# CHONSPQX/modulated-deform-conv

Hardware: AMD Instinct MI355X
Metric: fwd+bwd GSamples/s, MDCN2d 3x3 C=256 56x56 B=32; %HBM roofline (higher is better)
Workload: dtype f32; 1 GPU; ModulatedDeformConv2d 3x3, C_in=C_out=256, 56x56, deformable_group=1, fp32, B=32 per GPU, forward+backward (BASELINE.json configs[1]); global_batch=32, parallelism=dp1 batch-sharded

## Files before the change

modulated_deform_conv_amd/csrc/mfma_bwd_data.hip:

```cpp
#include "mfma_kernels.hpp"
#include "mfma_tile.hpp"
#include <algorithm>
#include <map>
#include <mutex>
#include <stdio.h>
#include <stdlib.h>

namespace mdconv {

namespace {

int grid_for(int64_t total) {
  int64_t b = (total + 255) / 256;
  return (int)(b > 8192 ? 8192 : (b < 1 ? 1 : b));
}

__device__ __forceinline__ void pack_wq_items(const Geom &g, int ochunks, int cblks, const float *__restrict__ w,
                                              float *__restrict__ wq, int64_t first, int64_t step) {
  const int64_t total = (int64_t)g.K * ochunks * cblks * 2 * 64;
  for (int64_t i = first; i < total; i += step) {
    int64_t r = i;
    const int lane = (int)(r & 63); r >>= 6;
    const int q = (int)(r & 1); r >>= 1;
    const int cblk = (int)(r % cblks); r /= cblks;
// ... 957 lines not shown
        }
      }
    }
    if (step > 0) {
      float *tp = tile + (r * 4) * (QT + 1) + (a - q0);
      tp[0] = cur.x; tp[QT + 1] = cur.y; tp[2 * (QT + 1)] = cur.z; tp[3 * (QT + 1)] = cur.w;
    }
    cur = nxt;
    nxt = make_float4(0.f, 0.f, 0.f, 0.f);
  }
  __syncthreads();
  for (int x = threadIdx.x; x < CW * (QT / 8); x += 256) {
    const int c = x / (QT / 8), qs8 = (x % (QT / 8)) * 8;
    float *dst = grad_input + ((int64_t)b * g.C + c) * g.S_i + q0 + qs8;
    const float *src = tile + c * (QT + 1) + qs8;
#pragma unroll
    for (int k = 0; k < 8; ++k)
      if (q0 + qs8 + k < g.S_i) dst[k] = g.acc_data ? dst[k] + src[k] : src[k];
  }
}

}

int pack_wq_f32(const Geom &g, const BwdDims &bd, const float *weight, float *wq, hipStream_t stream) {
  const int64_t total = (int64_t)g.K * bd.ochunks * bd.cblks_q * 2 * 64;
  hipLaunchKernelGGL(pack_wq_kernel, dim3(grid_for(total)), dim3(256), 0, stream, g, bd.ochunks,
                     bd.cblks_q, weight, wq);
  return check_launch("pack_wq");
}

int bwd_prep_f32(const Geom &g, const BwdDims &bd, const float *weight, float *wq, int *cnt, const float *x,
                 float *xt, hipStream_t stream) {
  const int64_t pack_total = (int64_t)g.K * bd.ochunks * bd.cblks_q * 2 * 64;
  const int64_t cnt_n = (int64_t)g.B * g.DG * bd.S_e;
  int nb_pack = grid_for(pack_total), nb_zero = grid_for(cnt_n);
  if (nb_pack > 512) nb_pack = 512;
  if (nb_zero > 256) nb_zero = 256;
  const int qtiles = (g.S_i + 31) / 32, ctiles = g.C / 32;
  const int64_t nb_t = xt ? (int64_t)qtiles * ctiles * g.B : 0;
  if (nb_t + nb_pack + nb_zero > 0x7fffffff) {
    int rc = pack_wq_f32(g, bd, weight, wq, stream);
    if (!rc) rc = csr_zero_f32(g, bd, cnt, stream);
    if (!rc && xt) rc = nchw_to_nhwc_f32(g, x, xt, stream);
    return rc;
  }
  hipLaunchKernelGGL(bwd_prep_kernel, dim3((unsigned)(nb_pack + nb_zero + nb_t)), dim3(256), 0, stream, g, bd.ochunks,
                     bd.cblks_q, weight, wq, cnt, cnt_n, x, xt, nb_pack, nb_zero, qtiles, ctiles);
  return check_launch("bwd_prep");
}

int num_cus() {
  static int n = 0;
  if (n == 0) {
    int dev = 0, v = 0;
    if (hipGetDevice(&dev) == hipSuccess &&
        hipDeviceGetAttribute(&v, hipDeviceAttributeMultiprocessorCount, dev) == hipSuccess && v > 0)
      n = v;
    else
      n = 256;
  }
  return n;
}

size_t bwd_data_lds_bytes(const Geom &g, const BwdDims &bd) {
  const int bnp = 32 * (4 / bd.waves_c);
  const int passes = bd.cblks_q / (2 * bd.waves_c);
  const size_t red = (size_t)bd.red_floats;
// ... 48 lines not shown
                       dim3(256), lds, stream,                                                  \
                       g, bd, (const float *)t.input, (const float *)t.grad_output, wq,         \
                       (const float *)t.offset, (const float *)t.mask, gcol,                    \
                       (float *)t.grad_offset, (float *)t.grad_mask, ga, bias_part, cnt, table, xt,        \
                       ntiles, n_full, n_tail, tpw);                                            \
  } while (0)
                                                \
#define LAUNCH_BD(ND, MOD, WC, QPQ)                                                             \
  do {                                                                                          \
    if (xt != nullptr && bd.cl_drain) LAUNCH_BD_(ND, MOD, WC, QPQ, true);                       \
    else LAUNCH_BD_(ND, MOD, WC, QPQ, false);                                                   \
  } while (0)
#define LAUNCH_BD2(ND, MOD)                                                                     \
  do {                                                                                          \
    const int nbatch = ND == 2 ? 4 : 8, nquads = bd.ochunks / 4;                                \
                   \
    const int qpq = (ND == 2 && g.G == 1 && nquads % nbatch == 0 && nquads / nbatch <= 2) ? nquads / nbatch : 0; \
    if (bd.waves_c == 4) {                                                                      \
      if (ND == 2 && qpq == 1) LAUNCH_BD(ND, MOD, 4, (ND == 2 ? 1 : 0));                        \
      else if (ND == 2 && qpq == 2) LAUNCH_BD(ND, MOD, 4, (ND == 2 ? 2 : 0));                   \
      else LAUNCH_BD(ND, MOD, 4, 0);                                                            \
    } else if (bd.waves_c == 2) LAUNCH_BD(ND, MOD, 2, 0);                                       \
    else LAUNCH_BD(ND, MOD, 1, 0);                                                              \
  } while (0)
  if (g.nd == 2) { if (g.modulated) LAUNCH_BD2(2, true); else LAUNCH_BD2(2, false); }
  else { if (g.modulated) LAUNCH_BD2(3, true); else LAUNCH_BD2(3, false); }
#undef LAUNCH_BD2
#undef LAUNCH_BD
#undef LAUNCH_BD_
  return check_launch("mfma_bwd_data");
}

int csr_zero_f32(const Geom &g, const BwdDims &bd, int *cnt, hipStream_t stream) {
  const int64_t cnt_n = (int64_t)g.B * g.DG * bd.S_e;
  hipLaunchKernelGGL(zero_int_kernel, dim3(grid_for(cnt_n)), dim3(256), 0, stream, cnt, cnt_n);
  return check_launch("zero_cnt");
}

int csr_build_f32(const Geom &g, const BwdDims &bd, const Tensors &t, int *cnt, int *rowptr,
                  void *entries, hipStream_t stream) {
  const int64_t samples = (int64_t)g.B * g.DG * g.K * g.S_o;
  int rc;
  hipLaunchKernelGGL(csr_scan_kernel, dim3((bd.S_e + kScanChunk - 1) / kScanChunk, g.B * g.DG), dim3(256), 0,
                     stream, bd.S_e, cnt, rowptr);
  if ((rc = check_launch("csr_scan"))) return rc;
  if (bd.sample_keyed) return csr_fill3d_f32(g, bd, t, cnt, rowptr, entries, stream);
#define LAUNCH_CSR(ND, MOD)                                                                     \
  hipLaunchKernelGGL((csr_fill_kernel<ND, MOD>), dim3(grid_for(samples)), dim3(256), 0, stream,  \
                     g, (const float *)t.offset, (const float *)t.mask, cnt, rowptr,            \
                     (int4 *)entries)
  if (g.modulated) LAUNCH_CSR(2, true); else LAUNCH_CSR(2, false);
#undef LAUNCH_CSR
  return check_launch("csr_fill");
}

int col2im_f32(const Geom &g, const BwdDims &bd, const Tensors &t, const float *gcol,
               const int *rowptr, const void *entries, float *sums, hipStream_t stream) {
  if (bd.sample_keyed) return col2im3d_f32(g, bd, t, gcol, rowptr, entries, sums, stream);
  const int qtiles = (g.S_i + 31) / 32;
  const dim3 grid(g.B * qtiles, 1);
#define LAUNCH_GG(ND, LPD)                                                                      \
  hipLaunchKernelGGL((col2im_gather_grouped_kernel<ND, LPD>), grid, dim3(256), 0, stream, g,    \
                     gcol, rowptr, (const int4 *)entries, (float *)t.grad_input)
#define LAUNCH_NARROW(ND, LPD)                                                                  \
  do {                                                                                          \
    const int qt = 4 * (64 / LPD) * kRun;                                                       \
    hipLaunchKernelGGL((col2im_gather_narrow_kernel<ND, LPD>), dim3(g.B * ((g.S_i + qt - 1) / qt)), \
// ... 22 lines not shown
```

modulated_deform_conv_amd/csrc/mfma_bwd_weight.hip:

```cpp
#include "mfma_kernels.hpp"
#include "mfma_tile.hpp"

namespace mdconv {

namespace {


template <int ND, bool PADN, int WR, int WC, int MB>
__global__ __launch_bounds__(256) void mfma_bwd_weight_kernel(Geom g, BwdDims bd,
                                                              const float *__restrict__ input,
                                                              const float *__restrict__ ga,
                                                              const int *__restrict__ table,
                                                              float *__restrict__ part) {
  static_assert(WR * WC == 4, "four waves");
  constexpr int NC = 1 << ND, NP = NC / 2;
  constexpr int BK = kBK;
  constexpr int RM = WR * MB * 32, CN = WC * 32;
  constexpr int CT = CN / 16;
  constexpr int kPitch = CN + 1;
  __shared__ __attribute__((aligned(16))) float Bs[2 * BK * kPitch];

  int id = blockIdx.x;
  const int cblk = id % bd.cblks; id /= bd.cblks;
  const int tap = id % g.K;
  const int mtile = id / g.K;
  const int split = blockIdx.y;
  const int c0 = cblk * CN;
  const int dg = min(c0, g.C - 1) / g.Cdg;

  const int tid = threadIdx.x, lane = tid & 63, kh = lane >> 5;
  const int wave = __builtin_amdgcn_readfirstlane(tid >> 6);
  const int wr = wave / WC, wcn = wave % WC;
  const int kk = tid & 15, sub = tid >> 4;

// ... 200 lines not shown
  float s = 0.f;
#pragma unroll
  for (int k = 0; k < kBiasSlices; ++k) s += stage[(size_t)k * g.O + o];
  grad_bias[o] = g.acc_w ? grad_bias[o] + s : s;
}

int grid_for(int64_t total) {
  int64_t b = (total + 255) / 256;
  return (int)(b > 8192 ? 8192 : (b < 1 ? 1 : b));
}

}

int mfma_bwd_weight_occupancy(int nd, bool padn, int wtile) {
  static int cache[2][2][2] = {};
  int &slot = cache[nd == 3][padn][wtile == 1];
  if (slot) return slot;
  int n = 0;
#define OCC_BW(ND, PADN, WR, WC, MB)                                                                           \
  (void)hipOccupancyMaxActiveBlocksPerMultiprocessor(                                                          \
      &n, reinterpret_cast<const void *>(&mfma_bwd_weight_kernel<ND, PADN, WR, WC, MB>), 256, 0)
#define OCC_BW2(ND, PADN) OCC_BW(ND, PADN, 4, 1, 2)
  if (nd == 2) { if (padn) OCC_BW2(2, true); else OCC_BW2(2, false); }
  else { if (padn) OCC_BW2(3, true); else OCC_BW2(3, false); }
#undef OCC_BW2
#undef OCC_BW
  (void)hipGetLastError();
  if (n <= 0) n = 4;
  slot = n;
  return n;
}

int mfma_bwd_weight_f32(const Geom &g, const BwdDims &bd, const Tensors &t, const float *ga,
                        const int *table, float *part, const float *bias_part, const float *xt,
                        hipStream_t stream) {
  const dim3 grid(bd.mtiles * g.K * bd.cblks, bd.splits);
  const bool padn = bd.Np != g.N;
  profile_mark(2, true, stream, bd.cl ? "mfma_bwd_weight_cl_kernel" : "mfma_bwd_weight_kernel");
  if (bd.cl) {
    const int rcl = mfma_bwd_weight_cl_launch(g, bd, xt, ga, table, part, stream);
    if (rcl) return rcl;
  } else {
#define LAUNCH_BW(ND, PADN, WR, WC, MB)                                                         \
  hipLaunchKernelGGL((mfma_bwd_weight_kernel<ND, PADN, WR, WC, MB>), grid, dim3(256), 0, stream, \
                     g, bd, (const float *)t.input, ga, table, part)
#define LAUNCH_BW2(ND, PADN) LAUNCH_BW(ND, PADN, 4, 1, 2)
  if (g.nd == 2) { if (padn) LAUNCH_BW2(2, true); else LAUNCH_BW2(2, false); }
  else { if (padn) LAUNCH_BW2(3, true); else LAUNCH_BW2(3, false); }
#undef LAUNCH_BW2
#undef LAUNCH_BW
  }
  profile_mark(2, false, stream);
  int rc = check_launch("mfma_bwd_weight");
  if (rc) return rc;
  hipLaunchKernelGGL(reduce_weight_kernel, dim3(grid_for((int64_t)g.K * g.O * g.Cg)), dim3(256), 0,
                     stream, g, bd, part, (float *)t.grad_weight);
  return check_launch("reduce_weight");
}

size_t grad_bias_stage_bytes(const Geom &g) { return (size_t)kBiasSlices * g.O * sizeof(float); }

int grad_bias_f32(const Geom &g, const BwdDims &bd, const float *bias_part, float *stage, float *grad_bias,
                  hipStream_t stream) {
  if (!g.with_bias) return MDCONV_OK;
  hipLaunchKernelGGL(grad_bias_stage1_kernel, dim3((g.O + 63) / 64, kBiasSlices), dim3(256), 0, stream, g,
                     bd.bias_tiles, bias_part, stage);
  int rc = check_launch("grad_bias_stage1");
  if (rc) return rc;
  hipLaunchKernelGGL(grad_bias_final_kernel, dim3((g.O + 255) / 256), dim3(256), 0, stream, g, stage, grad_bias);
  return check_launch("grad_bias_final");
}

}
```

modulated_deform_conv_amd/csrc/mfma_bwd_weight_cl.hip:

```cpp
#include "mfma_kernels.hpp"
#include "mfma_tile.hpp"

#include <stdlib.h>

namespace mdconv {

namespace {


template <int ND, bool PADN, int WR, int WC, int MB, int NBW>
__global__ __launch_bounds__(256, 1) void mfma_bwd_weight_cl_kernel(Geom g, BwdDims bd,
                                                                 const float *__restrict__ xt,
                                                                 const float *__restrict__ ga,
                                                                 const int *__restrict__ table,
                                                                 float *__restrict__ part) {
  static_assert(WR * WC == 4 && WC * NBW * 32 == 64, "four waves, 64 input channels");
  constexpr int NC = 1 << ND;
  constexpr int BK = kBK;
  constexpr int RM = WR * MB * 32, CN = WC * NBW * 32;
  constexpr int NH = CN / 64;
  constexpr int kPitch = CN + 1;
  __shared__ __attribute__((aligned(16))) float Bs[2 * BK * kPitch];

  const int per_split = gridDim.x;
  const int unit = xcd_remap(blockIdx.x + per_split * blockIdx.y, per_split * gridDim.y);
  const int split = unit / per_split;
  int id = unit - split * per_split;
  const int cblk = id % bd.cblks; id /= bd.cblks;
  const int tap = id % g.K;
  const int mtile = id / g.K;
  const int c0 = cblk * CN;

  const int tid = threadIdx.x, lane = tid & 63, kh = lane >> 5;
  const int wave = __builtin_amdgcn_readfirstlane(tid >> 6);
  const int wr = wave / WC, wcn = wave % WC;
  const int cq = tid & 15, kk = tid >> 4;

  const int pairs_total = bd.Np / 32;
  const int p_begin = split * bd.pairs_per_split;
  const int p_end = min(p_begin + bd.pairs_per_split, pairs_total);
  const int t_begin = 2 * p_begin, t_end = 2 * p_end;

  const rsrc_t r_xt = make_rsrc(xt, (size_t)g.B * g.S_i * g.C * sizeof(float));
  const int slab_bytes = bd.mblks * 2 * 64 * 16;
  const rsrc_t r_ga = make_rsrc(ga, (size_t)(bd.Np / 16) * slab_bytes);
  const int entry_bytes = 2 * NC * 4;
  const int dg = c0 / g.Cdg;
  const rsrc_t r_tab = make_rsrc(table + (size_t)(dg * g.K + tap) * bd.Np * (2 * NC),
                                 (size_t)bd.Np * entry_bytes);
  const int wo = mtile * RM + wr * MB * 32;
  const int a_voff = ((wo / 32) * 2 * 64 + lane) * 16;
  bool m_active = wo < g.O;
  if (g.G > 1) {
    const int cw = c0 + wcn * NBW * 32;
    const int o_lo = (min(cw, g.C - 1) / g.Cg) * g.Og;
    const int o_hi = (min(cw + NBW * 32 - 1, g.C - 1) / g.Cg + 1) * g.Og;
    m_active = m_active && wo < o_hi && wo + MB * 32 > o_lo;
  }
  const int t_voff = kk * entry_bytes;
  const int c_voff = (min(c0, g.C - CN) + cq * 4) * 4;
// ... 72 lines not shown
    load_tab(tabA, t_begin);
    load_tab(tabB, t_begin + 1);
    load_a(ra0, t_begin);
    gather(tabA);
    for (int t = t_begin; t < t_end; t += 2) {
      commit(tabA, t, Bs);
      __syncthreads();
      load_a(ra1, t + 1);
      gather(tabB);
      load_tab(tabA, min(t + 2, t_last));
      __builtin_amdgcn_sched_barrier(0);
      mma(ra0, Bs);
      commit(tabB, t + 1, Bs + BK * kPitch);
      __syncthreads();
      load_a(ra0, min(t + 2, t_last));
      gather(tabA);
      load_tab(tabB, min(t + 3, t_last));
      __builtin_amdgcn_sched_barrier(0);
      mma(ra1, Bs + BK * kPitch);
    }
  }

#pragma unroll
  for (int n = 0; n < NBW; ++n) {
    float *dst = part + ((size_t)(split * g.K + tap) * bd.OgpB) * bd.Cp + c0 + (wcn * NBW + n) * 32 + (lane & 31);
#pragma unroll
    for (int mb = 0; mb < MB; ++mb)
#pragma unroll
      for (int r = 0; r < 16; ++r) {
        const int o = wo + mb * 32 + (r & 3) + 8 * (r >> 2) + 4 * kh;
        dst[(size_t)o * bd.Cp] = acc[mb][n][r];
      }
  }
}


template <int ND, bool PADN, int MB>
__global__ __launch_bounds__(256) void mfma_bwd_weight_cl64_kernel(Geom g, BwdDims bd,
                                                                   const float *__restrict__ xt,
                                                                   const float *__restrict__ ga,
                                                                   const int *__restrict__ table,
                                                                   float *__restrict__ part) {
  constexpr int NC = 1 << ND;
  constexpr int SW = 2 * NC;
  constexpr int SP = 64;
  constexpr int kPitch = 65;
  constexpr int RM = 2 * MB * 32;
  constexpr int TPT = (SP * SW + 1023) / 1024;
  static_assert(TPT == 1, "one table piece per thread");
  __shared__ __attribute__((aligned(16))) float Bs[2 * SP * kPitch];
  __shared__ __attribute__((aligned(16))) int Ts[2 * SP * SW];

  const int per_split = gridDim.x;
  const int unit = xcd_remap(blockIdx.x + per_split * blockIdx.y, per_split * gridDim.y);
  const int split = unit / per_split;
  int id = unit - split * per_split;
  const int cblk = id % bd.cblks; id /= bd.cblks;
  const int tap = id % g.K;
  const int mtile = id / g.K;
  const int c0 = cblk * 64;

  const int tid = threadIdx.x, lane = tid & 63, kh = lane >> 5;
  const int wave = __builtin_amdgcn_readfirstlane(tid >> 6);
  const int wr = wave >> 1, wcn = wave & 1;
  const int cq = tid & 15, pg = tid >> 4;

// ... 150 lines not shown
#define MDCONV_CL_INSTANCE(ND, PADN, CALL)                                                                     \
  do {                                                                                                          \
    if (wtile == 1) { CALL##64(ND, PADN, 1); }                                                                  \
    else if (wtile == 2) { CALL##64(ND, PADN, 2); }                                                             \
    else { CALL(ND, PADN, 4, 1, 2, 2); }                                                                        \
  } while (0)
#define MDCONV_CL_DISPATCH(CALL)                                                                               \
  do {                                                                                                          \
    if (nd == 2) { if (padn) MDCONV_CL_INSTANCE(2, true, CALL); else MDCONV_CL_INSTANCE(2, false, CALL); }      \
    else { if (padn) MDCONV_CL_INSTANCE(3, true, CALL); else MDCONV_CL_INSTANCE(3, false, CALL); }              \
  } while (0)

int mfma_bwd_weight_cl_occupancy(int nd, bool padn, int wtile) {
  static int cache[2][2][4] = {};
  int &slot = cache[nd == 3][padn][wtile < 0 || wtile > 3 ? 3 : wtile];
  if (slot) return slot;
  int n = 0;
#define OCC_CL(ND, PADN, WR, WC, MB, NBW)                                                                      \
  (void)hipOccupancyMaxActiveBlocksPerMultiprocessor(                                                          \
      &n, reinterpret_cast<const void *>(&mfma_bwd_weight_cl_kernel<ND, PADN, WR, WC, MB, NBW>), 256, 0)
#define OCC_CL64(ND, PADN, MB)                                                                                 \
  (void)hipOccupancyMaxActiveBlocksPerMultiprocessor(                                                          \
      &n, reinterpret_cast<const void *>(&mfma_bwd_weight_cl64_kernel<ND, PADN, MB>), 256, 0)
  MDCONV_CL_DISPATCH(OCC_CL);
#undef OCC_CL64
#undef OCC_CL
  (void)hipGetLastError();
  if (n <= 0) n = 3;
  slot = n;
  return n;
}

int mfma_bwd_weight_cl_launch(const Geom &g, const BwdDims &bd, const float *xt, const float *ga,
                              const int *table, float *part, hipStream_t stream) {
  const dim3 grid(bd.mtiles * g.K * bd.cblks, bd.splits);
  const bool padn = bd.Np != g.N;
  const int nd = g.nd, wtile = bd.wtile;
#define LAUNCH_CL(ND, PADN, WR, WC, MB, NBW)                                                                   \
  hipLaunchKernelGGL((mfma_bwd_weight_cl_kernel<ND, PADN, WR, WC, MB, NBW>), grid, dim3(256), 0,               \
                     stream, g, bd, xt, ga, table, part)
#define LAUNCH_CL64(ND, PADN, MB)                                                                              \
  hipLaunchKernelGGL((mfma_bwd_weight_cl64_kernel<ND, PADN, MB>), grid, dim3(256), 0, stream, g, bd, xt, ga,   \
                     table, part)
  MDCONV_CL_DISPATCH(LAUNCH_CL);
#undef LAUNCH_CL64
#undef LAUNCH_CL
  return check_launch("mfma_bwd_weight_cl");
}

#undef MDCONV_CL_DISPATCH
#undef MDCONV_CL_INSTANCE

}
```

modulated_deform_conv_amd/csrc/mfma_kernels.hip:

```cpp
#include "mfma_kernels.hpp"
#include "mfma_tile.hpp"

#include <stdio.h>
#include <stdlib.h>
#include <string.h>

#include <atomic>
#include <mutex>
#include <vector>

namespace mdconv {

namespace {

std::atomic<bool> g_prof_on{false};
std::mutex g_prof_mu;
struct ProfPair { hipEvent_t a, b; };
constexpr int kProfSlots = 5;
std::vector<ProfPair> g_prof[kProfSlots];
size_t g_prof_used[kProfSlots] = {0, 0, 0, 0, 0};
const char *g_prof_name[kProfSlots] = {"", "", "", "", ""};

__global__ __launch_bounds__(256) void pack_weights_kernel(Geom g, PackDims pd,
                                                           const float *__restrict__ w,
// ... 52 lines not shown
  const bool words = bytes % 4 == 0 && ((uintptr_t)p & 3) == 0;
  const int64_t n = (int64_t)(words ? bytes / 4 : bytes / 2);
  const int64_t blocks = (n + 255) / 256;
  const dim3 grid((unsigned)(blocks > 8192 ? 8192 : blocks));
  if (words) hipLaunchKernelGGL(zero_words_kernel, grid, dim3(256), 0, s, (unsigned *)p, n);
  else hipLaunchKernelGGL(zero_halfwords_kernel, grid, dim3(256), 0, s, (unsigned short *)p, n);
  return check_launch("zero");
}

void profile_mark(int which, bool begin, hipStream_t stream, const char *name) {
  if (!g_prof_on.load(std::memory_order_relaxed) || which < 0 || which >= kProfSlots) return;
  std::lock_guard<std::mutex> lock(g_prof_mu);
  if (name) g_prof_name[which] = name;
  if (begin) {
    if (g_prof_used[which] == g_prof[which].size()) {
      ProfPair p;
      if (hipEventCreate(&p.a) != hipSuccess || hipEventCreate(&p.b) != hipSuccess) return;
      g_prof[which].push_back(p);
    }
    (void)hipEventRecord(g_prof[which][g_prof_used[which]].a, stream);
  } else if (g_prof_used[which] < g_prof[which].size()) {
    (void)hipEventRecord(g_prof[which][g_prof_used[which]].b, stream);
    ++g_prof_used[which];
  }
}

int pack_weights_f32(const Geom &g, const PackDims &pd, const float *weight, float *wp, float *wq,
                     hipStream_t stream) {
  const int64_t total = (int64_t)g.G * g.K * pd.Cgp * pd.Ogp;
  int blocks = (int)((total + 255) / 256);
  if (blocks > 4096) blocks = 4096;
  hipLaunchKernelGGL(pack_weights_kernel, dim3(blocks), dim3(256), 0, stream, g, pd, weight, wp, wq);
  return check_launch("pack_weights");
}

BwdDims bwd_dims(const Geom &g) {
  BwdDims bd;
  bd.Np = (g.N + 31) / 32 * 32;
  bd.cl = bwd_channels_last(g) ? 1 : 0;
  bd.wtile = 0;
  if (bd.cl) bd.wtile = g.O <= 64 ? 1 : (g.O <= 128 ? 2 : 3);
  const int rm = bd.cl ? (bd.wtile == 1 ? 64 : (bd.wtile == 2 ? 128 : 256)) : (bd.wtile ? 64 : 256);
  const int cn = bd.cl ? 64 : (bd.wtile ? 64 : 32);
  bd.OgpB = (g.O + rm - 1) / rm * rm;
  bd.mblks = bd.OgpB / 32;
  bd.mtiles = bd.OgpB / rm;
  bd.Cp = (g.C + cn - 1) / cn * cn;
  bd.cblks = bd.Cp / cn;
  const int col_tiles = bd.mtiles * g.K * bd.cblks;
  const int pairs = bd.Np / 32;
  const bool padn = bd.Np != g.N;
  const int occ = bd.cl ? mfma_bwd_weight_cl_occupancy(g.nd, padn, bd.wtile)
                        : mfma_bwd_weight_occupancy(g.nd, padn, bd.wtile);
  const int occ_run = bwd_fork_enabled() && occ > 1 ? occ - 1 : occ;
  const int slots = device_cus() * occ_run;
  int splits = slots / col_tiles;
  if (splits > pairs) splits = pairs;
  if (splits < 1) splits = 1;
  bd.pairs_per_split = (pairs + splits - 1) / splits;
  bd.splits = (pairs + bd.pairs_per_split - 1) / bd.pairs_per_split;
  static const bool debug_plan = getenv("MDCONV_DEBUG_PLAN") != nullptr;
  if (debug_plan)
    fprintf(stderr, "[mdconv] GEMM-2 plan: cl %d wtile %d col_tiles %d occ %d slots %d splits %d x %d pairs\n", bd.cl,
            bd.wtile, col_tiles, occ, slots, bd.splits, bd.pairs_per_split);
  bd.ochunks = (g.O + 63) / 64 * 4;
  bd.waves_c = g.C > 128 ? 4 : (g.C > 64 ? 2 : 1);
  for (;;) {
    bd.cblks_q = (g.C + 64 * bd.waves_c - 1) / (64 * bd.waves_c) * (2 * bd.waves_c);
    const int red_per_tap = 128 * (g.DG > 1 ? bd.cblks_q / (2 * bd.waves_c) : 1) * (g.nd + 1);
    const bool single_owner = g.DG == 1 && bd.waves_c == 1 && bd.cblks_q == 2;
    auto size_red = [&]() {
      bd.tap_group = 9;
      bd.red_floats = single_owner ? 0 : bd.tap_group * red_per_tap;
      if (bd.red_floats && bwd_data_lds_bytes(g, bd) > 80 * 1024) {
        bd.tap_group = 3;
        bd.red_floats = bd.tap_group * red_per_tap;
      }
    };
    {
      const int nbatch = g.nd == 2 ? 4 : 8, nquads = bd.ochunks / 4;
      const bool straight = g.nd == 2 && g.G == 1 && nquads % nbatch == 0 && nquads / nbatch <= 2;
      static const int bd_cl_env = getenv("MDCONV_BD_CL") ? atoi(getenv("MDCONV_BD_CL")) : -1;
      bd.cl_drain = bd.cl;
      size_red();
      if (bd.cl && straight && (bd_cl_env == 0 || (bd_cl_env < 0 && bwd_data_lds_bytes(g, bd) > 80 * 1024))) {
        bd.cl_drain = 0;
        size_red();
      }
    }
    if (bwd_data_lds_bytes(g, bd) <= kBwdDataLdsCap || bd.waves_c == 4) break;
    bd.waves_c *= 2;
  }
  const int nc = 1 << g.nd;
  size_t off = 0;
  bd.off_wq = off;   off += align_up((size_t)g.K * bd.ochunks * bd.cblks_q * 2 * 64 * 16);
  bd.off_ga = off;   off += align_up((size_t)bd.Np * bd.OgpB * sizeof(float));
  bd.off_table = off; off += align_up((size_t)g.DG * g.K * bd.Np * 2 * (1 << g.nd) * sizeof(int));
  bd.off_part = off; off += align_up((size_t)bd.splits * g.K * bd.OgpB * bd.Cp * sizeof(float));
  bd.off_gcol = off; off += align_up((size_t)g.B * g.C * g.K * g.S_o * sizeof(float));
  bd.sample_keyed = g.nd == 3 ? 1 : 0;
  bd.S_e = bd.sample_keyed ? hp_anchor_space(g) : g.S_i;
  bd.off_cnt = off;  off += align_up((size_t)g.B * g.DG * bd.S_e * sizeof(int));
  bd.off_rowptr = off; off += align_up((size_t)g.B * g.DG * (bd.S_e + 1) * sizeof(int));
  bd.off_entries = off; off += align_up((size_t)g.B * g.DG * g.K * g.S_o * (bd.sample_keyed ? 32 : (nc / 2) * 16));
  bd.bias_tiles = (g.N + 32 * (4 / bd.waves_c) - 1) / (32 * (4 / bd.waves_c));
  bd.off_bias = off; off += align_up((size_t)bd.bias_tiles * g.O * sizeof(float));
  bd.off_xt = off;   off += bd.cl ? align_up((size_t)g.B * g.S_i * g.C * sizeof(float)) : 0;
  static const int c2i_env = getenv("MDCONV_C2I3D") ? atoi(getenv("MDCONV_C2I3D")) : 2;
  bd.two_pass = bd.sample_keyed && c2i_env >= 2 ? 1 : 0;
  bd.off_sums = off; off += bd.two_pass ? align_up(col2im3d_sums_bytes(g)) : 0;
  bd.off_bstage = off; off += g.with_bias ? align_up(grad_bias_stage_bytes(g)) : 0;
  bd.off_end = off;
  return bd;
}

namespace {

size_t chunk_limit() {
  static size_t lim = 0;
  if (!lim) {
    lim = ((size_t)1 << 31) - (1 << 16);
    const char *e = getenv("MDCONV_CHUNK_LIMIT_BYTES");
    if (e && atoll(e) > 0 && (size_t)atoll(e) < lim) lim = (size_t)atoll(e);
  }
  return lim;
}

struct Plan {
  int Bc;
  bool half_io;
  Geom gc;
  size_t core_bytes;
  size_t off_w, off_b, off_x, off_off, off_m, off_go, off_out, off_gi, off_goff, off_gm, off_gw, off_gb;
  size_t total;
};
// ... 118 lines not shown
  g_forks.push_back({{dev, stream}, f});
  *out = f;
  return true;
}
int bwd_fork_mode() {
  static const int on = getenv("MDCONV_BWD_FORK") ? atoi(getenv("MDCONV_BWD_FORK")) : 1;
  return on;
}
bool bwd_fork_enabled() { return bwd_fork_mode() != 0; }

int backward_chunk_f32(const Geom &g, const Tensors &t, char *base, hipStream_t stream,
                       bool weights_final) {
  const BwdDims bd = bwd_dims(g);
  float *wq = (float *)(base + bd.off_wq);
  float *ga = (float *)(base + bd.off_ga);
  int *table = (int *)(base + bd.off_table);
  float *part = (float *)(base + bd.off_part);
  float *gcol = (float *)(base + bd.off_gcol);
  int *cnt = (int *)(base + bd.off_cnt), *rowptr = (int *)(base + bd.off_rowptr);
  void *entries = base + bd.off_entries;
  int rc;
  float *bias_part = g.with_bias ? (float *)(base + bd.off_bias) : nullptr;
  float *bstage = g.with_bias ? (float *)(base + bd.off_bstage) : nullptr;
  float *xt = bd.cl ? (float *)(base + bd.off_xt) : nullptr;
  if ((rc = bwd_prep_f32(g, bd, (const float *)t.weight, wq, cnt, (const float *)t.input, xt, stream))) return rc;
  profile_mark(1, true, stream, "mfma_bwd_data_kernel");
  rc = mfma_bwd_data_f32(g, bd, t, wq, gcol, ga, bias_part, cnt, table, xt, stream);
  profile_mark(1, false, stream);
  if (rc) return rc;
  Fork fk;
  const bool fork = bwd_fork_enabled() && get_fork(stream, &fk);
  hipStream_t gs = stream;
  auto gemm2 = [&](bool bias_here) {
    int r = mfma_bwd_weight_f32(g, bd, t, ga, table, part, bias_part, xt, stream);
    if (!r && bias_here) r = grad_bias_f32(g, bd, bias_part, bstage, (float *)t.grad_bias, stream);
    if (!r && !bias_here && g.with_bias && hipStreamWaitEvent(stream, fk.bias, 0) != hipSuccess) {
      set_error("backward fork failed");
      r = MDCONV_ELAUNCH;
    }
    if (!r && weights_final) r = record_weight_ready(stream);
    return r;
  };
  if (fork) {
    if (hipEventRecord(fk.fork, stream) != hipSuccess || hipStreamWaitEvent(fk.side, fk.fork, 0) != hipSuccess) {
      set_error("backward fork failed");
      return MDCONV_ELAUNCH;
    }
    gs = fk.side;
  } else {
    if ((rc = gemm2(true))) return rc;
  }
  const bool gemm2_first = fork && bwd_fork_mode() == 2;
  rc = MDCONV_OK;
  if (fork && g.with_bias) {
    rc = grad_bias_f32(g, bd, bias_part, bstage, (float *)t.grad_bias, gs);
    if (!rc && hipEventRecord(fk.bias, gs) != hipSuccess) { set_error("backward fork failed"); rc = MDCONV_ELAUNCH; }
  }
  if (!rc && gemm2_first) rc = gemm2(false);
  if (!rc) rc = csr_build_f32(g, bd, t, cnt, rowptr, entries, gs);
  if (!rc) {
    profile_mark(3, true, gs, bd.sample_keyed ? (bd.two_pass ? "col2im3d_sums_kernel" : "col2im3d_kernel") : "col2im_gather_kernel");
    rc = col2im_f32(g, bd, t, gcol, rowptr, entries, (float *)(base + bd.off_sums), gs);
    profile_mark(3, false, gs);
  }
  if (fork) {
    if (!rc && !gemm2_first) rc = gemm2(false);
    if ((hipEventRecord(fk.join, fk.side) != hipSuccess || hipStreamWaitEvent(stream, fk.join, 0) != hipSuccess) && !rc) {
// ... 822 lines not shown
```

modulated_deform_conv_amd/csrc/mfma_tile.hpp:

```cpp
#pragma once
#include "mdconv_common.hpp"

namespace mdconv {

typedef float f32x16 __attribute__((ext_vector_type(16)));

constexpr int kBK = 16;

struct PackDims {
  int Cgp;
  int Ogp;
  int BM;
};

inline PackDims pack_dims(const Geom &g) {
  PackDims pd;
  pd.BM = g.Og > 128 ? 256 : (g.Og > 64 ? 128 : 64);
  pd.Cgp = (g.Cg + 2 * kBK - 1) / (2 * kBK) * (2 * kBK);
  pd.Ogp = (g.Og + pd.BM - 1) / pd.BM * pd.BM;
  return pd;
}

__device__ __forceinline__ int xcd_remap(int bid, int n) {
  const int q = n >> 3, r = n & 7;
// ... 7 lines not shown
  const unsigned n = bytes > 0xfffffff0ull ? 0xfffffff0u : (unsigned)bytes;
  return __builtin_amdgcn_make_buffer_rsrc(const_cast<void *>(p), 0, (int)n, 0x00020000);
}
__device__ __forceinline__ float buf_load(rsrc_t r, int voff, int soff) {
  return __builtin_bit_cast(float, __builtin_amdgcn_raw_buffer_load_b32(r, voff, soff, 0));
}
struct F2bits { float x, y; };
__device__ __forceinline__ float2 buf_load2(rsrc_t r, int voff, int soff) {
  const F2bits f = __builtin_bit_cast(F2bits, __builtin_amdgcn_raw_buffer_load_b64(r, voff, soff, 0));
  return make_float2(f.x, f.y);
}
struct F4bits { float x, y, z, w; };
__device__ __forceinline__ float4 buf_load4(rsrc_t r, int voff, int soff) {
  const F4bits f = __builtin_bit_cast(F4bits, __builtin_amdgcn_raw_buffer_load_b128(r, voff, soff, 0));
  return make_float4(f.x, f.y, f.z, f.w);
}

template <int AUX = 0>
__device__ __forceinline__ void buf_store4(rsrc_t r, int voff, int soff, float a, float b, float c,
                                           float d) {
  typedef unsigned int u32x4 __attribute__((__vector_size__(4 * sizeof(unsigned int))));
  const u32x4 v = {__builtin_bit_cast(unsigned, a), __builtin_bit_cast(unsigned, b),
                   __builtin_bit_cast(unsigned, c), __builtin_bit_cast(unsigned, d)};
  __builtin_amdgcn_raw_buffer_store_b128(v, r, voff, soff, AUX);
}

struct BwdDims {
  int Np;
  int cl;
  int wtile;
  int OgpB, mblks, mtiles;
  int Cp, cblks;
  int splits, pairs_per_split;
  int ochunks;
  int waves_c, cblks_q;
  int bias_tiles;
  int red_floats;
  int tap_group;
  int cl_drain;
  int sample_keyed;
  int S_e;
  size_t off_wq, off_ga, off_table, off_part, off_gcol, off_cnt, off_rowptr, off_entries, off_bias,
      off_xt, off_sums, off_bstage, off_end;
  int two_pass;
};
BwdDims bwd_dims(const Geom &g);

#ifdef __HIPCC__
__device__ __forceinline__ void nchw_to_nhwc_tile(float (*t)[33], int C, int S, const float *__restrict__ x,
                                                  float *__restrict__ xt, int b, int c0, int q0) {
  const int tx = threadIdx.x & 31, ty = threadIdx.x >> 5;
  const float *src = x + ((size_t)b * C + c0) * S;
  float *dst = xt + ((size_t)b * S + q0) * C + c0;
#pragma unroll
  for (int r = ty; r < 32; r += 8) t[r][tx] = (q0 + tx < S) ? src[(size_t)r * S + q0 + tx] : 0.f;
  __syncthreads();
#pragma unroll
  for (int r = ty; r < 32; r += 8)
    if (q0 + r < S) dst[(size_t)r * C + tx] = t[tx][r];
}
#endif

int pack_weights_f32(const Geom &g, const PackDims &pd, const float *weight, float *wp, float *wq,
                     hipStream_t stream);
size_t fwd_tail_bytes(const Geom &g);
constexpr int kTailMaxPerCu = 5;
void fwd_tail_plan(const Geom &g, int tiles, int slots, int *full_tiles, int *ways, int *n_hi);
int fwd_tail_reduce_launch(int BM, int BN, const Geom &g, const float *part, const float *bias, float *output, int ntm,
                           int tail_tiles, int full_tiles, int ways, int n_hi, hipStream_t stream);
int mfma_forward_f32(const Geom &g, const PackDims &pd, const Tensors &t, const float *wp, float *part,
                     hipStream_t stream);
bool fwd_channels_last(const Geom &g);
size_t fwd_cl_bytes(const Geom &g);
int mfma_forward_cl_f32(const Geom &g, const PackDims &pd, const Tensors &t, const float *wp, float *part,
                        float *xt, hipStream_t stream);
int mfma_bwd_weight_f32(const Geom &g, const BwdDims &bd, const Tensors &t, const float *ga,
                        const int *table, float *part, const float *bias_part, const float *xt,
                        hipStream_t stream);
int mfma_bwd_weight_cl_launch(const Geom &g, const BwdDims &bd, const float *xt, const float *ga,
                              const int *table, float *part, hipStream_t stream);
int mfma_bwd_weight_cl_occupancy(int nd, bool padn, int wtile);
int mfma_bwd_weight_occupancy(int nd, bool padn, int wtile);
int device_cus();
bool bwd_channels_last(const Geom &g);
int nchw_to_nhwc_f32(const Geom &g, const float *x, float *xt, hipStream_t stream);
int pack_wq_f32(const Geom &g, const BwdDims &bd, const float *weight, float *wq, hipStream_t stream);
int bwd_prep_f32(const Geom &g, const BwdDims &bd, const float *weight, float *wq, int *cnt, const float *x,
                 float *xt, hipStream_t stream);
size_t grad_bias_stage_bytes(const Geom &g);
int grad_bias_f32(const Geom &g, const BwdDims &bd, const float *bias_part, float *stage, float *grad_bias,
                  hipStream_t stream);
size_t bwd_data_lds_bytes(const Geom &g, const BwdDims &bd);
constexpr size_t kBwdDataLdsCap = 150 * 1024;
int mfma_bwd_data_f32(const Geom &g, const BwdDims &bd, const Tensors &t, const float *wq,
                      float *gcol, float *ga, float *bias_part, int *cnt, int *table,
                      const float *xt, hipStream_t stream);
int csr_zero_f32(const Geom &g, const BwdDims &bd, int *cnt, hipStream_t stream);
int csr_build_f32(const Geom &g, const BwdDims &bd, const Tensors &t, int *cnt, int *rowptr,
                  void *entries, hipStream_t stream);
int col2im_f32(const Geom &g, const BwdDims &bd, const Tensors &t, const float *gcol,
               const int *rowptr, const void *entries, float *sums, hipStream_t stream);
int csr_fill3d_f32(const Geom &g, const BwdDims &bd, const Tensors &t, int *cursor,
                   const int *rowptr, void *entries, hipStream_t stream);
int col2im3d_f32(const Geom &g, const BwdDims &bd, const Tensors &t, const float *gcol,
                 const int *rowptr, const void *entries, float *sums, hipStream_t stream);
size_t col2im3d_sums_bytes(const Geom &g);

}
```

Before: 71.12 GSamples/s.

## Fuse split-K weight-gradient reduction into GEMM-2 via last-block ticket counters

```diff
diff --git a/modulated_deform_conv_amd/csrc/mfma_bwd_data.hip b/modulated_deform_conv_amd/csrc/mfma_bwd_data.hip
--- a/modulated_deform_conv_amd/csrc/mfma_bwd_data.hip
+++ b/modulated_deform_conv_amd/csrc/mfma_bwd_data.hip
@@ -1013,7 +1013,7 @@
 int bwd_prep_f32(const Geom &g, const BwdDims &bd, const float *weight, float *wq, int *cnt, const float *x,
                  float *xt, hipStream_t stream) {
   const int64_t pack_total = (int64_t)g.K * bd.ochunks * bd.cblks_q * 2 * 64;
-  const int64_t cnt_n = (int64_t)g.B * g.DG * bd.S_e;
+  const int64_t cnt_n = (int64_t)g.B * g.DG * bd.S_e + bd.tickets;
   int nb_pack = grid_for(pack_total), nb_zero = grid_for(cnt_n);
   if (nb_pack > 512) nb_pack = 512;
   if (nb_zero > 256) nb_zero = 256;
@@ -1128,7 +1128,7 @@
 }
 
 int csr_zero_f32(const Geom &g, const BwdDims &bd, int *cnt, hipStream_t stream) {
-  const int64_t cnt_n = (int64_t)g.B * g.DG * bd.S_e;
+  const int64_t cnt_n = (int64_t)g.B * g.DG * bd.S_e + bd.tickets;
   hipLaunchKernelGGL(zero_int_kernel, dim3(grid_for(cnt_n)), dim3(256), 0, stream, cnt, cnt_n);
   return check_launch("zero_cnt");
 }
diff --git a/modulated_deform_conv_amd/csrc/mfma_bwd_weight.hip b/modulated_deform_conv_amd/csrc/mfma_bwd_weight.hip
--- a/modulated_deform_conv_amd/csrc/mfma_bwd_weight.hip
+++ b/modulated_deform_conv_amd/csrc/mfma_bwd_weight.hip
@@ -1,5 +1,8 @@
 #include "mfma_kernels.hpp"
 #include "mfma_tile.hpp"
+
+#include <stdio.h>
+#include <stdlib.h>
 
 namespace mdconv {
 
@@ -266,13 +269,17 @@
 }
 
 int mfma_bwd_weight_f32(const Geom &g, const BwdDims &bd, const Tensors &t, const float *ga,
-                        const int *table, float *part, const float *bias_part, const float *xt,
+                        const int *table, float *part, int *tickets, const float *bias_part, const float *xt,
                         hipStream_t stream) {
   const dim3 grid(bd.mtiles * g.K * bd.cblks, bd.splits);
   const bool padn = bd.Np != g.N;
+  static const bool debug_plan = getenv("MDCONV_DEBUG_PLAN") != nullptr;
+  if (debug_plan)
+    fprintf(stderr, "[mdconv] GEMM-2 launch: cl %d wtile %d splits %d reduce %s\n", bd.cl, bd.wtile, bd.splits,
+            tickets ? "fused" : "kernel");
   profile_mark(2, true, stream, bd.cl ? "mfma_bwd_weight_cl_kernel" : "mfma_bwd_weight_kernel");
   if (bd.cl) {
-    const int rcl = mfma_bwd_weight_cl_launch(g, bd, xt, ga, table, part, stream);
+    const int rcl = mfma_bwd_weight_cl_launch(g, bd, xt, ga, table, part, tickets, (float *)t.grad_weight, stream);
     if (rcl) return rcl;
   } else {
 #define LAUNCH_BW(ND, PADN, WR, WC, MB)                                                         \
@@ -286,7 +293,7 @@
   }
   profile_mark(2, false, stream);
   int rc = check_launch("mfma_bwd_weight");
-  if (rc) return rc;
+  if (rc || tickets) return rc;
   hipLaunchKernelGGL(reduce_weight_kernel, dim3(grid_for((int64_t)g.K * g.O * g.Cg)), dim3(256), 0,
                      stream, g, bd, part, (float *)t.grad_weight);
   return check_launch("reduce_weight");
diff --git a/modulated_deform_conv_amd/csrc/mfma_bwd_weight_cl.hip b/modulated_deform_conv_amd/csrc/mfma_bwd_weight_cl.hip
--- a/modulated_deform_conv_amd/csrc/mfma_bwd_weight_cl.hip
+++ b/modulated_deform_conv_amd/csrc/mfma_bwd_weight_cl.hip
@@ -13,7 +13,8 @@
                                                                  const float *__restrict__ xt,
                                                                  const float *__restrict__ ga,
                                                                  const int *__restrict__ table,
-                                                                 float *__restrict__ part) {
+                                                                 float *__restrict__ part, int *__restrict__ tickets,
+                                                                 float *__restrict__ grad_weight) {
   static_assert(WR * WC == 4 && WC * NBW * 32 == 64, "four waves, 64 input channels");
   constexpr int NC = 1 << ND;
   constexpr int BK = kBK;
@@ -164,6 +165,78 @@
         dst[(size_t)o * bd.Cp] = acc[mb][n][r];
       }
   }
+
+  if (tickets == nullptr) return;
+  __builtin_amdgcn_fence(__ATOMIC_RELEASE, "agent");
+  __syncthreads();
+  int *flag = reinterpret_cast<int *>(Bs);
+  if (tid == 0) *flag = __hip_atomic_fetch_add(tickets + (mtile * g.K + tap) * bd.cblks + cblk, 1, __ATOMIC_RELAXED,
+                                               __HIP_MEMORY_SCOPE_AGENT);
+  __syncthreads();
+  if (*flag != bd.splits - 1) return;
+  __builtin_amdgcn_fence(__ATOMIC_ACQUIRE, "agent");
+  constexpr int kRows = 2;
+  static_assert(RM % (16 * kRows) == 0, "whole steps");
+  const int stride = g.K * bd.OgpB * bd.Cp * 4;
+  const rsrc_t r_part = make_rsrc(part, (size_t)bd.splits * stride);
+  const int c = c0 + (tid & 15) * 4;
+  const int n8 = bd.splits & ~7, has4 = (bd.splits & 4) != 0, n1 = bd.splits & 3;
+  auto add4 = [](float4 &s, const float4 &a) { s.x += a.x; s.y += a.y; s.z += a.z; s.w += a.w; };
+  auto tree4 = [](const float4 &a, const float4 &b, const float4 &c4, const float4 &d) {
+    return make_float4((a.x + b.x) + (c4.x + d.x), (a.y + b.y) + (c4.y + d.y), (a.z + b.z) + (c4.z + d.z),
+                       (a.w + b.w) + (c4.w + d.w));
+  };
+  for (int row0 = tid >> 4; row0 < RM; row0 += 16 * kRows) {
+    const int voff = ((tap * bd.OgpB + mtile * RM + row0) * bd.Cp + c) * 4, row_step = 16 * bd.Cp * 4;
+    float4 s4[kRows];
+#pragma unroll
+    for (int k = 0; k < kRows; ++k) s4[k] = make_float4(0.f, 0.f, 0.f, 0.f);
+    for (int sp = 0; sp < n8; sp += 8) {
+      float4 a[kRows][8];
+#pragma unroll
+      for (int k = 0; k < kRows; ++k)
+#pragma unroll
+        for (int u = 0; u < 8; ++u) a[k][u] = buf_load4(r_part, voff + k * row_step, (sp + u) * stride);
+#pragma unroll
+      for (int k = 0; k < kRows; ++k) {
+        const float4 lo = tree4(a[k][0], a[k][1], a[k][2], a[k][3]), hi = tree4(a[k][4], a[k][5], a[k][6], a[k][7]);
+        s4[k].x += lo.x + hi.x; s4[k].y += lo.y + hi.y; s4[k].z += lo.z + hi.z; s4[k].w += lo.w + hi.w;
+      }
+    }
+    {
+      float4 a[kRows][7];
+#pragma unroll
+      for (int k = 0; k < kRows; ++k)
+#pragma unroll
+        for (int u = 0; u < 7; ++u) {
+          const bool on = u < 4 ? has4 : u - 4 < n1;
+          const int sp = u < 4 ? n8 + u : n8 + 4 * has4 + u - 4;
+          a[k][u] = buf_load4(r_part, on ? voff + k * row_step : 0x7ffffff0, on ? sp * stride : 0);
+        }
+#pragma unroll
+      for (int k = 0; k < kRows; ++k) {
+        if (has4) add4(s4[k], tree4(a[k][0], a[k][1], a[k][2], a[k][3]));
+#pragma unroll
+        for (int u = 0; u < 3; ++u)
+          if (u < n1) add4(s4[k], a[k][4 + u]);
+      }
+    }
+#pragma unroll
+    for (int k = 0; k < kRows; ++k) {
+      const int o = mtile * RM + row0 + 16 * k;
+      if (o >= g.O) continue;
+      const int cg0 = (o / g.Og) * g.Cg;
+      const float sv[4] = {s4[k].x, s4[k].y, s4[k].z, s4[k].w};
+#pragma unroll
+      for (int j = 0; j < 4; ++j) {
+        const int cl = c + j - cg0;
+        if (cl >= 0 && cl < g.Cg) {
+          float *dst = grad_weight + ((int64_t)o * g.Cg + cl) * g.K + tap;
+          *dst = g.acc_w ? *dst + sv[j] : sv[j];
+        }
+      }
+    }
+  }
 }
 
 
@@ -380,13 +453,13 @@
 }
 
 int mfma_bwd_weight_cl_launch(const Geom &g, const BwdDims &bd, const float *xt, const float *ga,
-                              const int *table, float *part, hipStream_t stream) {
+                              const int *table, float *part, int *tickets, float *grad_weight, hipStream_t stream) {
   const dim3 grid(bd.mtiles * g.K * bd.cblks, bd.splits);
   const bool padn = bd.Np != g.N;
   const int nd = g.nd, wtile = bd.wtile;
 #define LAUNCH_CL(ND, PADN, WR, WC, MB, NBW)                                                                   \
   hipLaunchKernelGGL((mfma_bwd_weight_cl_kernel<ND, PADN, WR, WC, MB, NBW>), grid, dim3(256), 0,               \
-                     stream, g, bd, xt, ga, table, part)
+                     stream, g, bd, xt, ga, table, part, tickets, grad_weight)
 #define LAUNCH_CL64(ND, PADN, MB)                                                                              \
   hipLaunchKernelGGL((mfma_bwd_weight_cl64_kernel<ND, PADN, MB>), grid, dim3(256), 0, stream, g, bd, xt, ga,   \
                      table, part)
diff --git a/modulated_deform_conv_amd/csrc/mfma_kernels.hip b/modulated_deform_conv_amd/csrc/mfma_kernels.hip
--- a/modulated_deform_conv_amd/csrc/mfma_kernels.hip
+++ b/modulated_deform_conv_amd/csrc/mfma_kernels.hip
@@ -108,6 +108,14 @@
   if (blocks > 4096) blocks = 4096;
   hipLaunchKernelGGL(pack_weights_kernel, dim3(blocks), dim3(256), 0, stream, g, pd, weight, wp, wq);
   return check_launch("pack_weights");
+}
+
+static bool gemm2_reduce_fused() {
+  static const bool fused = [] {
+    const char *e = getenv("MDCONV_GEMM2_REDUCE");
+    return !(e && strcmp(e, "kernel") == 0);
+  }();
+  return fused;
 }
 
 BwdDims bwd_dims(const Geom &g) {
@@ -176,7 +184,8 @@
   bd.off_gcol = off; off += align_up((size_t)g.B * g.C * g.K * g.S_o * sizeof(float));
   bd.sample_keyed = g.nd == 3 ? 1 : 0;
   bd.S_e = bd.sample_keyed ? hp_anchor_space(g) : g.S_i;
-  bd.off_cnt = off;  off += align_up((size_t)g.B * g.DG * bd.S_e * sizeof(int));
+  bd.tickets = bd.cl && bd.wtile == 3 && gemm2_reduce_fused() ? col_tiles : 0;
+  bd.off_cnt = off;  off += align_up(((size_t)g.B * g.DG * bd.S_e + bd.tickets) * sizeof(int));
   bd.off_rowptr = off; off += align_up((size_t)g.B * g.DG * (bd.S_e + 1) * sizeof(int));
   bd.off_entries = off; off += align_up((size_t)g.B * g.DG * g.K * g.S_o * (bd.sample_keyed ? 32 : (nc / 2) * 16));
   bd.bias_tiles = (g.N + 32 * (4 / bd.waves_c) - 1) / (32 * (4 / bd.waves_c));
@@ -361,7 +370,8 @@
   const bool fork = bwd_fork_enabled() && get_fork(stream, &fk);
   hipStream_t gs = stream;
   auto gemm2 = [&](bool bias_here) {
-    int r = mfma_bwd_weight_f32(g, bd, t, ga, table, part, bias_part, xt, stream);
+    int r = mfma_bwd_weight_f32(g, bd, t, ga, table, part, bd.tickets ? cnt + (size_t)g.B * g.DG * bd.S_e : nullptr,
+                                bias_part, xt, stream);
     if (!r && bias_here) r = grad_bias_f32(g, bd, bias_part, bstage, (float *)t.grad_bias, stream);
     if (!r && !bias_here && g.with_bias && hipStreamWaitEvent(stream, fk.bias, 0) != hipSuccess) {
       set_error("backward fork failed");
diff --git a/modulated_deform_conv_amd/csrc/mfma_tile.hpp b/modulated_deform_conv_amd/csrc/mfma_tile.hpp
--- a/modulated_deform_conv_amd/csrc/mfma_tile.hpp
+++ b/modulated_deform_conv_amd/csrc/mfma_tile.hpp
@@ -74,6 +74,7 @@
   size_t off_wq, off_ga, off_table, off_part, off_gcol, off_cnt, off_rowptr, off_entries, off_bias,
       off_xt, off_sums, off_bstage, off_end;
   int two_pass;
+  int tickets;
 };
 BwdDims bwd_dims(const Geom &g);
 
@@ -106,10 +107,10 @@
 int mfma_forward_cl_f32(const Geom &g, const PackDims &pd, const Tensors &t, const float *wp, float *part,
                         float *xt, hipStream_t stream);
 int mfma_bwd_weight_f32(const Geom &g, const BwdDims &bd, const Tensors &t, const float *ga,
-                        const int *table, float *part, const float *bias_part, const float *xt,
+                        const int *table, float *part, int *tickets, const float *bias_part, const float *xt,
                         hipStream_t stream);
 int mfma_bwd_weight_cl_launch(const Geom &g, const BwdDims &bd, const float *xt, const float *ga,
-                              const int *table, float *part, hipStream_t stream);
+                              const int *table, float *part, int *tickets, float *grad_weight, hipStream_t stream);
 int mfma_bwd_weight_cl_occupancy(int nd, bool padn, int wtile);
 int mfma_bwd_weight_occupancy(int nd, bool padn, int wtile);
 int device_cus();
```

New measurement: 69.00 GSamples/s, median of 2. 0.97x the previous value.

## Fuse split-K weight-gradient reduction into last-arriving block via atomic tickets

Applied to the files above, without the earlier changes.

```diff
diff --git a/modulated_deform_conv_amd/csrc/mfma_bwd_data.hip b/modulated_deform_conv_amd/csrc/mfma_bwd_data.hip
--- a/modulated_deform_conv_amd/csrc/mfma_bwd_data.hip
+++ b/modulated_deform_conv_amd/csrc/mfma_bwd_data.hip
@@ -1013,7 +1013,7 @@
 int bwd_prep_f32(const Geom &g, const BwdDims &bd, const float *weight, float *wq, int *cnt, const float *x,
                  float *xt, hipStream_t stream) {
   const int64_t pack_total = (int64_t)g.K * bd.ochunks * bd.cblks_q * 2 * 64;
-  const int64_t cnt_n = (int64_t)g.B * g.DG * bd.S_e;
+  const int64_t cnt_n = (int64_t)g.B * g.DG * bd.S_e + bd.tickets;
   int nb_pack = grid_for(pack_total), nb_zero = grid_for(cnt_n);
   if (nb_pack > 512) nb_pack = 512;
   if (nb_zero > 256) nb_zero = 256;
@@ -1128,7 +1128,7 @@
 }
 
 int csr_zero_f32(const Geom &g, const BwdDims &bd, int *cnt, hipStream_t stream) {
-  const int64_t cnt_n = (int64_t)g.B * g.DG * bd.S_e;
+  const int64_t cnt_n = (int64_t)g.B * g.DG * bd.S_e + bd.tickets;
   hipLaunchKernelGGL(zero_int_kernel, dim3(grid_for(cnt_n)), dim3(256), 0, stream, cnt, cnt_n);
   return check_launch("zero_cnt");
 }
diff --git a/modulated_deform_conv_amd/csrc/mfma_bwd_weight.hip b/modulated_deform_conv_amd/csrc/mfma_bwd_weight.hip
--- a/modulated_deform_conv_amd/csrc/mfma_bwd_weight.hip
+++ b/modulated_deform_conv_amd/csrc/mfma_bwd_weight.hip
@@ -267,12 +267,12 @@
 
 int mfma_bwd_weight_f32(const Geom &g, const BwdDims &bd, const Tensors &t, const float *ga,
                         const int *table, float *part, const float *bias_part, const float *xt,
-                        hipStream_t stream) {
+                        int *tickets, hipStream_t stream) {
   const dim3 grid(bd.mtiles * g.K * bd.cblks, bd.splits);
   const bool padn = bd.Np != g.N;
   profile_mark(2, true, stream, bd.cl ? "mfma_bwd_weight_cl_kernel" : "mfma_bwd_weight_kernel");
   if (bd.cl) {
-    const int rcl = mfma_bwd_weight_cl_launch(g, bd, xt, ga, table, part, stream);
+    const int rcl = mfma_bwd_weight_cl_launch(g, bd, xt, ga, table, part, (float *)t.grad_weight, tickets, stream);
     if (rcl) return rcl;
   } else {
 #define LAUNCH_BW(ND, PADN, WR, WC, MB)                                                         \
@@ -286,7 +286,7 @@
   }
   profile_mark(2, false, stream);
   int rc = check_launch("mfma_bwd_weight");
-  if (rc) return rc;
+  if (rc || bd.fused_reduce) return rc;
   hipLaunchKernelGGL(reduce_weight_kernel, dim3(grid_for((int64_t)g.K * g.O * g.Cg)), dim3(256), 0,
                      stream, g, bd, part, (float *)t.grad_weight);
   return check_launch("reduce_weight");
diff --git a/modulated_deform_conv_amd/csrc/mfma_bwd_weight_cl.hip b/modulated_deform_conv_amd/csrc/mfma_bwd_weight_cl.hip
--- a/modulated_deform_conv_amd/csrc/mfma_bwd_weight_cl.hip
+++ b/modulated_deform_conv_amd/csrc/mfma_bwd_weight_cl.hip
@@ -6,6 +6,67 @@
 namespace mdconv {
 
 namespace {
+
+__device__ __forceinline__ float4 add4(const float4 &a, const float4 &b) {
+  return make_float4(a.x + b.x, a.y + b.y, a.z + b.z, a.w + b.w);
+}
+
+template <int RM>
+__device__ __forceinline__ void reduce_tile_in_order(const Geom &g, const BwdDims &bd, const float *part,
+                                                     float *__restrict__ grad_weight, int wave, int tap, int o0, int c0) {
+  constexpr int R = 2;
+  const int lane = __builtin_amdgcn_mbcnt_hi(~0u, __builtin_amdgcn_mbcnt_lo(~0u, 0u));
+  const int tid = wave * 64 + lane;
+  const int c = c0 + (tid & 15) * 4;
+  const int stride = g.K * bd.OgpB * bd.Cp * 4, row = 16 * bd.Cp * 4;
+  const rsrc_t r_part = make_rsrc(part, (size_t)bd.splits * stride);
+#pragma unroll 1
+  for (int r0 = tid >> 4; r0 < RM; r0 += 16 * R) {
+    const int voff = ((tap * bd.OgpB + o0 + r0) * bd.Cp + c) * 4;
+    auto ld4 = [&](int j, int sp) { return buf_load4(r_part, voff, j * row + sp * stride); };
+    float4 s[R];
+#pragma unroll
+    for (int j = 0; j < R; ++j) s[j] = make_float4(0.f, 0.f, 0.f, 0.f);
+    int sp = 0;
+    for (; sp + 8 <= bd.splits; sp += 8) {
+      float4 a[R][8];
+#pragma unroll
+      for (int j = 0; j < R; ++j)
+#pragma unroll
+        for (int u = 0; u < 8; ++u) a[j][u] = ld4(j, sp + u);
+#pragma unroll
+      for (int j = 0; j < R; ++j)
+        s[j] = add4(s[j], add4(add4(add4(a[j][0], a[j][1]), add4(a[j][2], a[j][3])),
+                               add4(add4(a[j][4], a[j][5]), add4(a[j][6], a[j][7]))));
+    }
+    for (; sp + 4 <= bd.splits; sp += 4) {
+      float4 a[R][4];
+#pragma unroll
+      for (int j = 0; j < R; ++j)
+#pragma unroll
+        for (int u = 0; u < 4; ++u) a[j][u] = ld4(j, sp + u);
+#pragma unroll
+      for (int j = 0; j < R; ++j) s[j] = add4(s[j], add4(add4(a[j][0], a[j][1]), add4(a[j][2], a[j][3])));
+    }
+    for (; sp < bd.splits; ++sp)
+#pragma unroll
+      for (int j = 0; j < R; ++j) s[j] = add4(s[j], ld4(j, sp));
+#pragma unroll
+    for (int j = 0; j < R; ++j) {
+      const int o = o0 + r0 + 16 * j;
+      if (o >= g.O) continue;
+      const int cb = (o / g.Og) * g.Cg;
+      const float v[4] = {s[j].x, s[j].y, s[j].z, s[j].w};
+#pragma unroll
+      for (int e = 0; e < 4; ++e) {
+        const int cl = c + e - cb;
+        if (cl < 0 || cl >= g.Cg) continue;
+        float *dst = grad_weight + ((int64_t)o * g.Cg + cl) * g.K + tap;
+        *dst = g.acc_w ? *dst + v[e] : v[e];
+      }
+    }
+  }
+}
 
 
 template <int ND, bool PADN, int WR, int WC, int MB, int NBW>
@@ -13,7 +74,9 @@
                                                                  const float *__restrict__ xt,
                                                                  const float *__restrict__ ga,
                                                                  const int *__restrict__ table,
-                                                                 float *__restrict__ part) {
+                                                                 float *__restrict__ part,
+                                                                 float *__restrict__ grad_weight,
+                                                                 int *__restrict__ tickets) {
   static_assert(WR * WC == 4 && WC * NBW * 32 == 64, "four waves, 64 input channels");
   constexpr int NC = 1 << ND;
   constexpr int BK = kBK;
@@ -21,11 +84,13 @@
   constexpr int NH = CN / 64;
   constexpr int kPitch = CN + 1;
   __shared__ __attribute__((aligned(16))) float Bs[2 * BK * kPitch];
+  __shared__ int ticket;
 
   const int per_split = gridDim.x;
   const int unit = xcd_remap(blockIdx.x + per_split * blockIdx.y, per_split * gridDim.y);
   const int split = unit / per_split;
-  int id = unit - split * per_split;
+  const int col_tile = unit - split * per_split;
+  int id = col_tile;
   const int cblk = id % bd.cblks; id /= bd.cblks;
   const int tap = id % g.K;
   const int mtile = id / g.K;
@@ -164,6 +229,17 @@
         dst[(size_t)o * bd.Cp] = acc[mb][n][r];
       }
   }
+
+  __threadfence();
+  __syncthreads();
+  if (bd.splits > 1) {
+    if (wave == 0 && __builtin_amdgcn_mbcnt_lo(~0u, 0u) == 0 && __builtin_amdgcn_mbcnt_hi(~0u, 0u) == 0)
+      ticket = atomicAdd(tickets + col_tile, 1);
+    __syncthreads();
+    if (ticket != bd.splits - 1) return;
+  }
+  __threadfence();
+  reduce_tile_in_order<RM>(g, bd, part, grad_weight, wave, tap, mtile * RM, c0);
 }
 
 
@@ -380,13 +456,14 @@
 }
 
 int mfma_bwd_weight_cl_launch(const Geom &g, const BwdDims &bd, const float *xt, const float *ga,
-                              const int *table, float *part, hipStream_t stream) {
+                              const int *table, float *part, float *grad_weight, int *tickets,
+                              hipStream_t stream) {
   const dim3 grid(bd.mtiles * g.K * bd.cblks, bd.splits);
   const bool padn = bd.Np != g.N;
   const int nd = g.nd, wtile = bd.wtile;
 #define LAUNCH_CL(ND, PADN, WR, WC, MB, NBW)                                                                   \
   hipLaunchKernelGGL((mfma_bwd_weight_cl_kernel<ND, PADN, WR, WC, MB, NBW>), grid, dim3(256), 0,               \
-                     stream, g, bd, xt, ga, table, part)
+                     stream, g, bd, xt, ga, table, part, grad_weight, tickets)
 #define LAUNCH_CL64(ND, PADN, MB)                                                                              \
   hipLaunchKernelGGL((mfma_bwd_weight_cl64_kernel<ND, PADN, MB>), grid, dim3(256), 0, stream, g, bd, xt, ga,   \
                      table, part)
diff --git a/modulated_deform_conv_amd/csrc/mfma_kernels.hip b/modulated_deform_conv_amd/csrc/mfma_kernels.hip
--- a/modulated_deform_conv_amd/csrc/mfma_kernels.hip
+++ b/modulated_deform_conv_amd/csrc/mfma_kernels.hip
@@ -135,6 +135,8 @@
   if (splits < 1) splits = 1;
   bd.pairs_per_split = (pairs + splits - 1) / splits;
   bd.splits = (pairs + bd.pairs_per_split - 1) / bd.pairs_per_split;
+  bd.fused_reduce = bd.cl && bd.wtile == 3 ? 1 : 0;
+  bd.tickets = bd.fused_reduce ? col_tiles : 0;
   static const bool debug_plan = getenv("MDCONV_DEBUG_PLAN") != nullptr;
   if (debug_plan)
     fprintf(stderr, "[mdconv] GEMM-2 plan: cl %d wtile %d col_tiles %d occ %d slots %d splits %d x %d pairs\n", bd.cl,
@@ -176,7 +178,9 @@
   bd.off_gcol = off; off += align_up((size_t)g.B * g.C * g.K * g.S_o * sizeof(float));
   bd.sample_keyed = g.nd == 3 ? 1 : 0;
   bd.S_e = bd.sample_keyed ? hp_anchor_space(g) : g.S_i;
-  bd.off_cnt = off;  off += align_up((size_t)g.B * g.DG * bd.S_e * sizeof(int));
+  bd.off_cnt = off;
+  bd.off_tickets = off + (size_t)g.B * g.DG * bd.S_e * sizeof(int);
+  off += align_up(((size_t)g.B * g.DG * bd.S_e + bd.tickets) * sizeof(int));
   bd.off_rowptr = off; off += align_up((size_t)g.B * g.DG * (bd.S_e + 1) * sizeof(int));
   bd.off_entries = off; off += align_up((size_t)g.B * g.DG * g.K * g.S_o * (bd.sample_keyed ? 32 : (nc / 2) * 16));
   bd.bias_tiles = (g.N + 32 * (4 / bd.waves_c) - 1) / (32 * (4 / bd.waves_c));
@@ -361,7 +365,7 @@
   const bool fork = bwd_fork_enabled() && get_fork(stream, &fk);
   hipStream_t gs = stream;
   auto gemm2 = [&](bool bias_here) {
-    int r = mfma_bwd_weight_f32(g, bd, t, ga, table, part, bias_part, xt, stream);
+    int r = mfma_bwd_weight_f32(g, bd, t, ga, table, part, bias_part, xt, (int *)(base + bd.off_tickets), stream);
     if (!r && bias_here) r = grad_bias_f32(g, bd, bias_part, bstage, (float *)t.grad_bias, stream);
     if (!r && !bias_here && g.with_bias && hipStreamWaitEvent(stream, fk.bias, 0) != hipSuccess) {
       set_error("backward fork failed");
diff --git a/modulated_deform_conv_amd/csrc/mfma_tile.hpp b/modulated_deform_conv_amd/csrc/mfma_tile.hpp
--- a/modulated_deform_conv_amd/csrc/mfma_tile.hpp
+++ b/modulated_deform_conv_amd/csrc/mfma_tile.hpp
@@ -63,6 +63,8 @@
   int OgpB, mblks, mtiles;
   int Cp, cblks;
   int splits, pairs_per_split;
+  int fused_reduce;
+  int tickets;
   int ochunks;
   int waves_c, cblks_q;
   int bias_tiles;
@@ -73,6 +75,7 @@
   int S_e;
   size_t off_wq, off_ga, off_table, off_part, off_gcol, off_cnt, off_rowptr, off_entries, off_bias,
       off_xt, off_sums, off_bstage, off_end;
+  size_t off_tickets;
   int two_pass;
 };
 BwdDims bwd_dims(const Geom &g);
@@ -107,9 +110,10 @@
                         float *xt, hipStream_t stream);
 int mfma_bwd_weight_f32(const Geom &g, const BwdDims &bd, const Tensors &t, const float *ga,
                         const int *table, float *part, const float *bias_part, const float *xt,
-                        hipStream_t stream);
+                        int *tickets, hipStream_t stream);
 int mfma_bwd_weight_cl_launch(const Geom &g, const BwdDims &bd, const float *xt, const float *ga,
-                              const int *table, float *part, hipStream_t stream);
+                              const int *table, float *part, float *grad_weight, int *tickets,
+                              hipStream_t stream);
 int mfma_bwd_weight_cl_occupancy(int nd, bool padn, int wtile);
 int mfma_bwd_weight_occupancy(int nd, bool padn, int wtile);
 int device_cus();
```

Result: slower. 70.97 GSamples/s before, 68.16 GSamples/s after (-4.0%).
